# ubisoft/ubisoft-laforge-msmd

Hardware: AMD Instinct MI355X
Metric: FLAME frames/sec on 4s@16kHz clips (whole job; MSMD.forward motion-coefficient frames) (higher is better)
Workload: dtype bf16; 1 GPU; configs[1]: MSMD.forward, batch=32 x 4 s clips per GPU, wav2vec2-base encoder + 8-layer motion decoder, eval-mode, synthetic closed-form weights; batch_per_gpu=32, frames_per_clip=100, parallelism=dp1 (independent clips, no collective), launch=one hipGraph replay per step (the batch sits in the captured input buffers)

## Files before the change

### include/msmd_hip.h

```cpp
#ifndef MSMD_HIP_H
#define MSMD_HIP_H

#include <stdint.h>

#ifdef __cplusplus
extern "C" {
#endif

#define MSMD_F32 0
#define MSMD_BF16 1
#define MSMD_F16 2
#define MSMD_F16X2 3

#define MSMD_ACT_NONE 0
#define MSMD_ACT_GELU 1
#define MSMD_ACT_ELU 2

typedef void* msmd_stream_t;

int msmd_abi_version(void);
#define MSMD_GEMM_VARIANT(v) ((v) << 8)
#define MSMD_GEMM_WRITE_THROUGH (1 << 16)
#define MSMD_GEMM_PAIRED_STORES (1 << 17)
#define MSMD_GEMM_STAGGER (1 << 18)
#define MSMD_GEMM_ONE_TILE_PER_WORKGROUP (1 << 19)
#define MSMD_GEMM_NO_256_TILE (1 << 20)
#define MSMD_GEMM_W_BELOW_32 (1 << 21)

int msmd_spin_us(float us, long* ticks_out, msmd_stream_t stream);

int msmd_gemm(const void* A, const void* W, const float* bias, const void* residual, void* C,
              int M, int N, int K, int in_dtype, int out_dtype,
              long lda, int rows_per_batch, long a_batch_stride, long ldw, long ldc, long ldr, int act,
              int batch, long strideA, long strideW, long strideC, long strideBias, long strideR,
              msmd_stream_t stream);

int msmd_gemm_ln(const void* A, const void* W, const float* bias, const void* residual, void* C, int M, int N, int K,
                 int in_dtype, int out_dtype, long lda, long ldw, long ldc, long ldr, int act, const float* a_stats,
                 const float* w_colsum, const float* r_stats, const float* r_gamma, const float* r_beta,
                 float* stats_out, int slab_in, int slab_out, float eps, msmd_stream_t stream);

int msmd_gemm_ex(const void* A, const void* W, const float* bias, const void* residual, void* C, int M, int N, int K,
                 int in_dtype, int out_dtype, long lda, int rows_per_batch, long a_batch_stride, long ldw, long ldc,
                 long ldr, int act, int batch, long strideA, long strideW, long strideC, long strideBias, long strideR,
                 void* z_out, float p_drop, const unsigned long* rng_state, unsigned int site, msmd_stream_t stream);

int msmd_gemm_route(const void* A, const void* W, const float* bias, const void* residual, void* C, int M, int N, int K,
                    int in_dtype, int out_dtype, long lda, int rows_per_batch, long a_batch_stride, long ldw, long ldc,
                    long ldr, int act, int batch, long strideA, long strideW, long strideC, long strideBias, long strideR,
                    void* z_out, float p_drop, const unsigned long* rng_state, unsigned int site, msmd_stream_t stream);
int msmd_gemm_ln_route(const void* A, const void* W, const float* bias, const void* residual, void* C, int M, int N, int K,
                       int in_dtype, int out_dtype, long lda, long ldw, long ldc, long ldr, int act, const float* a_stats,
                       const float* w_colsum, const float* r_stats, const float* r_gamma, const float* r_beta,
                       float* stats_out, int slab_in, int slab_out, float eps, msmd_stream_t stream);

int msmd_gemm_actbwd(const void* A, const void* W, const void* Z, void* C, int M, int N, int K, int in_dtype, int out_dtype,
                     long lda, long ldw, int act, float p_drop, const unsigned long* rng_state, unsigned int site,
                     msmd_stream_t stream);

int msmd_gemm_batched2(const void* A, const void* W, void* C, int M, int N, int K, int in_dtype, int out_dtype,
                       long lda, long ldw, long ldc, int batch_outer, long strideA_o, long strideW_o, long strideC_o,
                       int batch_inner, long strideA_i, long strideW_i, long strideC_i, msmd_stream_t stream);

int msmd_gemm_tn(const void* A, const void* B, float* C, float* colsum, int M, int N, int K, long lda, long ldb,
                 long ldc, int batch, long strideA, long strideB, long strideC, int b_rows_per_window,
                 long b_window_stride, int accumulate, void* ws, long ws_bytes, msmd_stream_t stream);
long msmd_gemm_tn_workspace(int M, int N, int K, int batch);

int msmd_layernorm(const void* x, const void* residual, const float* gamma, const float* beta,
                   const float* post_add, void* y, int rows, int cols, float eps, int act,
                   int in_dtype, int out_dtype, msmd_stream_t stream);
int msmd_layernorm_pre(const void* x, const float* pre_gamma, const float* pre_beta, const void* residual,
                       const float* gamma, const float* beta, void* y, int rows, int cols, float eps, int dtype,
                       msmd_stream_t stream);

int msmd_layernorm_f16x2(const float* x, const float* residual, const float* gamma, const float* beta,
                         const float* post_add, float* y, void* y_split, int rows, int cols, float eps, int act,
                         msmd_stream_t stream);

int msmd_split_f16x2(const float* x, void* y, long rows, int cols, long ldx, int cols_out, msmd_stream_t stream);
int msmd_unsplit_f16x2(const void* x, float* y, long rows, int cols, int cols_in, long ldy, msmd_stream_t stream);

int msmd_attention_prefetch(const void* Q, const void* K, const void* V, void* O, int B, int H, int Tq, int Tk,
                            long q_bstride, long q_tstride, long k_bstride, long k_tstride, long v_bstride,
                            long v_tstride, long o_bstride, long o_tstride, float scale, const uint8_t* mask, int dtype,
                            const void* const* prefetch_ptrs, const long* prefetch_bytes, int n_prefetch,
                            msmd_stream_t stream);
// ... 273 lines not shown
```

### ubisoft-laforge-msmd_amd/csrc/gemm.hip

```cpp
#include "common.h"
#include <atomic>
#include <utility>

struct GemmArgs {
  const void* A; const void* W; const float* bias; const void* R; void* C;
  int M, N, K;
  long lda; int rows_per_batch; long a_batch_stride; long ldw, ldc, ldr;
  int act; int vec_ok; float inv_rpb;
  long strideA, strideW, strideC, strideBias, strideR;
  int mt, nt;
  int batch_inner; long strideA2, strideW2, strideC2;
  void* Z; float p_drop; const unsigned long* rng; unsigned site;
  int xn;
  int flags;
  const float* a_stats = nullptr; int a_nt = 0; const float* w_colsum = nullptr;
  const float* r_stats = nullptr; int r_nt = 0; const float* r_gamma = nullptr; const float* r_beta = nullptr;
  float* stats_out = nullptr; float ln_eps = 1e-5f;
  int stagger_ticks = 0;
};

enum : int {
  GF_WRITE_THROUGH = 1, GF_PAIRED_STORES = 2, GF_STAGGER = 4,
  GF_ACT_BWD = 8,
  GF_ONE_TILE = 16, GF_NO_256 = 32,
  GF_W_BELOW_32 = 64,
};
struct GemmActWord { int act, hint, flags; };
static constexpr GemmActWord gemm_unpack_act(int act) {
  return {act & 0xff, (act >> 8) & 0xff, ((act >> 16) & 7) | (((act >> 19) & 7) << 4)};
}
static_assert(gemm_unpack_act(MSMD_GEMM_WRITE_THROUGH).flags == GF_WRITE_THROUGH && gemm_unpack_act(MSMD_GEMM_PAIRED_STORES).flags == GF_PAIRED_STORES &&
              gemm_unpack_act(MSMD_GEMM_STAGGER).flags == GF_STAGGER && gemm_unpack_act(MSMD_GEMM_ONE_TILE_PER_WORKGROUP).flags == GF_ONE_TILE &&
              gemm_unpack_act(MSMD_GEMM_NO_256_TILE).flags == GF_NO_256 && gemm_unpack_act(MSMD_GEMM_W_BELOW_32).flags == GF_W_BELOW_32 && gemm_unpack_act(~0).flags == (0x7f & ~GF_ACT_BWD),
              "internal flag bits follow include/msmd_hip.h; no bit of `act` sets the internal one");
enum : int {
  GV_GENERIC = 0,
  GV_SPLIT_128 = 1, GV_SPLIT_64 = 5,
  GV_64_DEEP = 9, GV_64 = 12,
  GV_256x64 = 14,
  GV_192 = 15,
  GV_128 = 17,
  GV_64x128 = 18,
  GV_128_AB = 13, GV_128_ONE_AB = 66,
  GV_256 = 80,
};

enum GemmEpi : int { EPI_ALL = 0, EPI_PLAIN = 1, EPI_LN_OPERAND = 2, EPI_LN_RESIDUAL = 3 };
constexpr int ACT_RUNTIME = -1;
constexpr int epia(GemmEpi e, int act) { return e + 10 * (1 + act); }
constexpr GemmEpi epia_family(int code) { return (GemmEpi)(code % 10); }
constexpr int epia_act(int code) { return code / 10 - 1; }

template <typename T> struct Mfma;
template <> struct Mfma<bf16_t> {
  static __device__ __forceinline__ void run(const u32x4& a, const u32x4& b, f32x4& acc) {
    acc = __builtin_amdgcn_mfma_f32_16x16x32_bf16(__builtin_bit_cast(bf16x8, a), __builtin_bit_cast(bf16x8, b),
                                                  acc, 0, 0, 0);
  }
};
template <> struct Mfma<f16_t> {
  static __device__ __forceinline__ void run(const u32x4& a, const u32x4& b, f32x4& acc) {
    acc = __builtin_amdgcn_mfma_f32_16x16x32_f16(__builtin_bit_cast(f16x8, a), __builtin_bit_cast(f16x8, b), acc, 0, 0, 0);
  }
};
template <> struct Mfma<float> {
  static __device__ __forceinline__ void run(const u32x4& a, const u32x4& b, f32x4& acc) {
#pragma unroll
// ... 208 lines not shown
      }
    }
  }
}

template <int FM>
__device__ __forceinline__ void ln_issue(const float* stats, int nt, int M, int m_base, int fr, int fq, f32x2 (&raw)[FM][4]) {
#pragma unroll
  for (int j = 0; j < FM; ++j) {
    const f32x2* sp = (const f32x2*)stats + min(m_base + j * 16 + fr, M - 1);
#pragma unroll
    for (int q = 0; q < 4; ++q) raw[j][q] = fq + 4 * q < nt ? sp[(long)(fq + 4 * q) * M] : f32x2{0.f, 0.f};
  }
}

template <int FM>
__device__ __forceinline__ void ln_finish(const float* stats, int nt, int M, int m_base, int fr, int fq, const f32x2 (&raw)[FM][4],
                                          float inv_cols, float eps, float (&mu)[FM], float (&rs)[FM]) {
#pragma unroll
  for (int j = 0; j < FM; ++j) {
    float S = (raw[j][0][0] + raw[j][1][0]) + (raw[j][2][0] + raw[j][3][0]);
    float Q = (raw[j][0][1] + raw[j][1][1]) + (raw[j][2][1] + raw[j][3][1]);
    if (nt > 16) {
      const f32x2* sp = (const f32x2*)stats + min(m_base + j * 16 + fr, M - 1);
      for (int t = 16 + fq; t < nt; t += 4) { const f32x2 w = sp[(long)t * M]; S += w[0]; Q += w[1]; }
    }
    S += __shfl_xor(S, 16, 64); S += __shfl_xor(S, 32, 64);
    Q += __shfl_xor(Q, 16, 64); Q += __shfl_xor(Q, 32, 64);
    mu[j] = S * inv_cols;
    rs[j] = rsqrtf(fmaxf(Q * inv_cols - mu[j] * mu[j], 0.f) + eps);
  }
}

template <typename TO, int FM, int FN> struct LnResOps { f32x4 bv[FN], xv[FN], yv[FN]; typename Vec4T<TO>::type rr[FM][FN]; };
template <typename TO, int FM, int FN>
__device__ __forceinline__ void ln_res_issue(const GemmArgs& p, int m_base, int n_base, int fr, int fq, LnResOps<TO, FM, FN>& o) {
  typedef typename Vec4T<TO>::type V4;
  const int n = n_base + fq * 4;
#pragma unroll
  for (int i = 0; i < FN; ++i) o.bv[i] = *(const f32x4*)(p.bias + n + i * 16);
#pragma unroll
  for (int j = 0; j < FM; ++j) {
    const TO* rp = (const TO*)p.R + (long)min(m_base + j * 16 + fr, p.M - 1) * p.ldr + n;
#pragma unroll
    for (int i = 0; i < FN; ++i) o.rr[j][i] = *(const V4*)(rp + i * 16);
  }
  if (p.r_stats) {
#pragma unroll
    for (int i = 0; i < FN; ++i) { o.xv[i] = *(const f32x4*)(p.r_gamma + n + i * 16); o.yv[i] = *(const f32x4*)(p.r_beta + n + i * 16); }
  } else {
#pragma unroll
    for (int i = 0; i < FN; ++i) { o.xv[i] = f32x4{1.f, 1.f, 1.f, 1.f}; o.yv[i] = f32x4{0.f, 0.f, 0.f, 0.f}; }
  }
}

template <typename TO, int FM, int FN, int MODE, int ACT = -1, bool EARLY = false>
__device__ __forceinline__ void gemm_epilogue_ln(const GemmArgs& p, const f32x4 (&acc)[FN][FM], int m_base, int n_base,
                                                 int fr, int fq, const f32x2 (&raw)[FM][4], const LnResOps<TO, FM, FN>* early = nullptr) {
  static_assert((FN == 4 || FN == 2) && (FM >= 2 && FM <= 4), "one wave = one statistics slab of 16 FN columns, 2 to 4 fragment rows");
  constexpr int SLAB = FN * 16;
  constexpr int IB = FM == 3 ? 2 : FN;
  typedef typename Vec4T<TO>::type V4;
  const int n = n_base + fq * 4;
  float mu[FM], rs[FM];
#pragma unroll
  for (int j = 0; j < FM; ++j) { mu[j] = 0.f; rs[j] = 1.f; }
  if constexpr (MODE == 1) ln_finish<FM>(p.a_stats, p.a_nt, p.M, m_base, fr, fq, raw, 1.0f / (float)p.K, p.ln_eps, mu, rs);
  else if (p.r_stats) ln_finish<FM>(p.r_stats, p.r_nt, p.M, m_base, fr, fq, raw, 1.0f / (float)p.N, p.ln_eps, mu, rs);
  float rowS[FM], rowQ[FM], tS[FM], tQ[FM], prS[FM], prQ[FM];
#pragma unroll
  for (int j = 0; j < FM; ++j) rowS[j] = rowQ[j] = tS[j] = tQ[j] = prS[j] = prQ[j] = 0.f;
  const bool odd = fq & 1;
  const bool pair = sizeof(TO) == 2 && (p.flags & GF_PAIRED_STORES);
#pragma unroll
  for (int i0 = 0; i0 < FN; i0 += IB) {
    f32x4 bv[IB], xv[IB], yv[IB];
    V4 rr[FM][IB];
    if constexpr (EARLY) {
      static_assert(MODE == 2 && IB == FN, "the early operands are the LayerNorm-residual form's, all fragment columns at once");
#pragma unroll
      for (int ii = 0; ii < IB; ++ii) {
        bv[ii] = early->bv[ii]; xv[ii] = early->xv[ii]; yv[ii] = early->yv[ii];
#pragma unroll
        for (int j = 0; j < FM; ++j) rr[j][ii] = early->rr[j][ii];
      }
    } else {
#pragma unroll
      for (int ii = 0; ii < IB; ++ii) bv[ii] = *(const f32x4*)(p.bias + n + (i0 + ii) * 16);
      if constexpr (MODE == 1) {
#pragma unroll
        for (int ii = 0; ii < IB; ++ii) xv[ii] = *(const f32x4*)(p.w_colsum + n + (i0 + ii) * 16);
      } else {
#pragma unroll
        for (int j = 0; j < FM; ++j) {
          const TO* rp = (const TO*)p.R + (long)min(m_base + j * 16 + fr, p.M - 1) * p.ldr + n;
#pragma unroll
          for (int ii = 0; ii < IB; ++ii) rr[j][ii] = *(const V4*)(rp + (i0 + ii) * 16);
        }
        if (p.r_stats) {
#pragma unroll
          for (int ii = 0; ii < IB; ++ii) { xv[ii] = *(const f32x4*)(p.r_gamma + n + (i0 + ii) * 16); yv[ii] = *(const f32x4*)(p.r_beta + n + (i0 + ii) * 16); }
        } else {
#pragma unroll
          for (int ii = 0; ii < IB; ++ii) { xv[ii] = f32x4{1.f, 1.f, 1.f, 1.f}; yv[ii] = f32x4{0.f, 0.f, 0.f, 0.f}; }
        }
      }
    }
#pragma unroll
    for (int ii = 0; ii < IB; ++ii) {
      const int i = i0 + ii;
      V4 o[FM];
#pragma unroll
      for (int j = 0; j < FM; ++j) {
        float v[4];
#pragma unroll
        for (int e = 0; e < 4; ++e) {
          float x = acc[i][j][e];
// ... 126 lines not shown
    for (int j = 0; j < FM; ++j) acc[i][j] = f32x4{0.f, 0.f, 0.f, 0.f};

  const int nk = (p.K + BKE - 1) / BKE;
  load_global(0);
  store_lds(0);
  __syncthreads();
  for (int kt = 0; kt < nk; ++kt) {
    const int cur = kt & 1;
    if (kt + 1 < nk) load_global((kt + 1) * BKE);
    const unsigned char* sa = smem + cur * (BM + BN) * 128;
    const unsigned char* sw = sa + BM * 128;
#pragma unroll
    for (int g = 0; g < 2; ++g) {
      u32x4 fx[FM], fw[FN];
#pragma unroll
      for (int j = 0; j < FM; ++j) fx[j] = *(const u32x4*)(sa + lds_off(wm + j * 16 + fr, g * 4 + fq));
#pragma unroll
      for (int i = 0; i < FN; ++i) fw[i] = *(const u32x4*)(sw + lds_off(wn + i * 16 + fr, g * 4 + fq));
#pragma unroll
      for (int i = 0; i < FN; ++i)
#pragma unroll
        for (int j = 0; j < FM; ++j) Mfma<T>::run(fw[i], fx[j], acc[i][j]);
    }
    if (kt + 1 < nk) store_lds(cur ^ 1);
    __syncthreads();
  }

  gemm_epilogue<TO, FM, FN>(p, acc, z, m0 + wm, n0 + wn, fr, fq);
}

typedef __attribute__((address_space(3))) void lds_void_t;
typedef __attribute__((address_space(1))) const void gbl_void_t;

template <typename TO, int BM, int BN, int WM, int WN, int NSTAGE, bool PIPE = false, typename TI = bf16_t, int EPIA = 0>
__global__ __launch_bounds__(WM * WN * 64, (WM * WN == 8 && NSTAGE * (BM + BN) * 128 <= 80 * 1024 && (epia_family(EPIA) != EPI_ALL || BM * BN <= 128 * 128)) ? 4 : 1) void gemm2_kernel(const GemmArgs p) {
  constexpr int EPI = epia_family(EPIA), ACTK = epia_act(EPIA);
  constexpr int NW = WM * WN, NT = NW * 64;
  constexpr int STAGE = (BM + BN) * 128;
  constexpr int LPT = (BM + BN) * 8 / NT;
  constexpr int FM = BM / WM / 16, FN = BN / WN / 16;
  static_assert((BM + BN) * 8 % NT == 0, "tile chunks must divide over the threads");
  extern __shared__ __attribute__((aligned(16))) unsigned char smem[];

  const int pid = blockIdx.x;
  const int xcd = pid & 7, slot = pid >> 3;
  const int xm_n = 8 / p.xn, ntx = (p.nt + p.xn - 1) / p.xn;
  const int m_tile = (slot / ntx) * xm_n + (xcd % xm_n), n_tile = (slot % ntx) * p.xn + xcd / xm_n;
  if (m_tile >= p.mt || n_tile >= p.nt) return;
  const int z = blockIdx.z;
  const int zo = z / p.batch_inner, zi = z % p.batch_inner;
  const bf16_t* __restrict__ A = (const bf16_t*)p.A + zo * p.strideA + zi * p.strideA2;
  const bf16_t* __restrict__ W = (const bf16_t*)p.W + zo * p.strideW + zi * p.strideW2;
  const int m0 = m_tile * BM, n0 = n_tile * BN;
  const int tid = threadIdx.x, lane = tid & 63, wid = tid >> 6;

  const bf16_t* src[LPT];
#pragma unroll
  for (int i = 0; i < LPT; ++i) {
    const int id = (i * NW + wid) * 64 + lane;
    const int row = id >> 3, phys = id & 7;
    const int c = phys ^ ((row >> 1) & 7);
    if (row < BM) {
      const int m = min(m0 + row, p.M - 1);
      src[i] = A + a_row_offset(p, m) + c * 8;
    } else {
      const int n = min(n0 + row - BM, p.N - 1);
      src[i] = W + (long)n * p.ldw + c * 8;
    }
  }
  auto issue = [&](int kt, int stage) {
#pragma unroll
    for (int i = 0; i < LPT; ++i)
      __builtin_amdgcn_global_load_lds((gbl_void_t*)(src[i] + kt * 64),
                                       (lds_void_t*)(smem + stage * STAGE + (i * NW + wid) * 1024), 16, 0, 0);
  };

  const int wm = (wid / WN) * (BM / WM), wn = (wid % WN) * (BN / WN);
  const int fr = lane & 15, fq = lane >> 4;
  f32x4 acc[FN][FM];
#pragma unroll
  for (int i = 0; i < FN; ++i)
#pragma unroll
    for (int j = 0; j < FM; ++j) acc[i][j] = f32x4{0.f, 0.f, 0.f, 0.f};

  const int nk = p.K / 64;
  constexpr bool LNK = (BN == 128 || BN == 64) && WN == 2 && (FM == 2 || FM == 3) && sizeof(TO) == 2;
  constexpr bool LN_LATE = FM == 3;
  constexpr bool EARLY_OPS = LNK && EPI == 3 && NW == 4 && BM == 64 && BN == 128;
  f32x2 lnraw[(LNK && !LN_LATE) ? FM : 1][4];
  std::conditional_t<EARLY_OPS, LnResOps<TO, FM, FN>, char> early;
  (void)early;
  if constexpr (EARLY_OPS) {
    if (p.r_stats) ln_issue<FM>(p.r_stats, p.r_nt, p.M, m0 + wm, fr, fq, lnraw);
    ln_res_issue<TO, FM, FN>(p, m0 + wm, n0 + wn, fr, fq, early);
  }
#pragma unroll
  for (int s = 0; s < NSTAGE - 1; ++s)
    if (s < nk) issue(s, s);
  if (p.stagger_ticks > 0 && ((pid >> 8) & 1) && pid < 512) {
    const unsigned long t0 = __builtin_amdgcn_s_memrealtime();
    while ((long)(__builtin_amdgcn_s_memrealtime() - t0) < p.stagger_ticks) __builtin_amdgcn_s_sleep(16);
  }
  if constexpr (LNK && !LN_LATE && EPI != 1 && !EARLY_OPS) {
    if (EPI == 2 || (EPI == 0 && p.a_stats)) ln_issue<FM>(p.a_stats, p.a_nt, p.M, m0 + wm, fr, fq, lnraw);
    else if (p.r_stats) ln_issue<FM>(p.r_stats, p.r_nt, p.M, m0 + wm, fr, fq, lnraw);
  }
  int stage = 0;
  for (int kt = 0; kt < nk; ++kt) {
    if (kt + NSTAGE - 2 < nk) asm volatile("s_waitcnt vmcnt(%0)" ::"n"((NSTAGE - 2) * LPT) : "memory");
    else asm volatile("s_waitcnt vmcnt(0)" ::: "memory");
    __builtin_amdgcn_s_barrier();
    if (kt + NSTAGE - 1 < nk) issue(kt + NSTAGE - 1, (stage + NSTAGE - 1) % NSTAGE);
    const unsigned char* sa = smem + stage * STAGE;
    const unsigned char* sw = sa + BM * 128;
    if constexpr (PIPE) {
      u32x4 fx[2][FM], fw[2][FN];
#pragma unroll
      for (int g = 0; g < 2; ++g) {
#pragma unroll
        for (int j = 0; j < FM; ++j) fx[g][j] = *(const u32x4*)(sa + lds_off(wm + j * 16 + fr, g * 4 + fq));
#pragma unroll
        for (int i = 0; i < FN; ++i) fw[g][i] = *(const u32x4*)(sw + lds_off(wn + i * 16 + fr, g * 4 + fq));
      }
      __builtin_amdgcn_sched_barrier(0);
#pragma unroll
      for (int g = 0; g < 2; ++g) {
#pragma unroll
        for (int i = 0; i < FN; ++i)
#pragma unroll
          for (int j = 0; j < FM; ++j) Mfma<TI>::run(fw[g][i], fx[g][j], acc[i][j]);
        __builtin_amdgcn_sched_barrier(0);
      }
    } else {
#pragma unroll
      for (int g = 0; g < 2; ++g) {
        u32x4 fx[FM], fw[FN];
#pragma unroll
        for (int j = 0; j < FM; ++j) fx[j] = *(const u32x4*)(sa + lds_off(wm + j * 16 + fr, g * 4 + fq));
#pragma unroll
        for (int i = 0; i < FN; ++i) fw[i] = *(const u32x4*)(sw + lds_off(wn + i * 16 + fr, g * 4 + fq));
#pragma unroll
        for (int i = 0; i < FN; ++i)
#pragma unroll
          for (int j = 0; j < FM; ++j) Mfma<TI>::run(fw[i], fx[j], acc[i][j]);
      }
    }
    stage = (stage + 1 == NSTAGE) ? 0 : stage + 1;
  }
  int tid_e = tid;
  if constexpr (LN_LATE) asm volatile("" : "+v"(tid_e));
  const int wm_e = ((tid_e >> 6) / WN) * (BM / WM), wn_e = ((tid_e >> 6) % WN) * (BN / WN);
  const int fr_e = tid_e & 15, fq_e = (tid_e & 63) >> 4;
  auto run_epilogue = [&]() {
    if constexpr (EPI == 1) { gemm_epilogue<TO, FM, FN, false, true, ACTK>(p, acc, z, m0 + wm_e, n0 + wn_e, fr_e, fq_e); return; }
    if constexpr (LNK && !LN_LATE && EPI == 2) { gemm_epilogue_ln<TO, FM, FN, 1, ACTK>(p, acc, m0 + wm_e, n0 + wn_e, fr_e, fq_e, lnraw); return; }
    if constexpr (EARLY_OPS) { gemm_epilogue_ln<TO, FM, FN, 2, ACTK, true>(p, acc, m0 + wm_e, n0 + wn_e, fr_e, fq_e, lnraw, &early); return; }
    if constexpr (LNK && !LN_LATE && EPI == 3) { gemm_epilogue_ln<TO, FM, FN, 2, ACTK>(p, acc, m0 + wm_e, n0 + wn_e, fr_e, fq_e, lnraw); return; }
    if constexpr (LNK && LN_LATE && (EPI == 2 || EPI == 3)) {
      f32x2 late[FM][4];
      if constexpr (EPI == 2) ln_issue<FM>(p.a_stats, p.a_nt, p.M, m0 + wm_e, fr_e, fq_e, late);
      else if (p.r_stats) ln_issue<FM>(p.r_stats, p.r_nt, p.M, m0 + wm_e, fr_e, fq_e, late);
      gemm_epilogue_ln<TO, FM, FN, EPI - 1, ACTK>(p, acc, m0 + wm_e, n0 + wn_e, fr_e, fq_e, late);
      return;
    }
    if constexpr (LNK && !LN_LATE) {
      if (p.a_stats) { gemm_epilogue_ln<TO, FM, FN, 1, ACTK>(p, acc, m0 + wm_e, n0 + wn_e, fr_e, fq_e, lnraw); return; }
      if (p.r_stats || p.stats_out) { gemm_epilogue_ln<TO, FM, FN, 2, ACTK>(p, acc, m0 + wm_e, n0 + wn_e, fr_e, fq_e, lnraw); return; }
    }
    if constexpr (LNK && LN_LATE) {
      if (p.a_stats || p.r_stats || p.stats_out) {
        f32x2 late[FM][4];
        if (p.a_stats) ln_issue<FM>(p.a_stats, p.a_nt, p.M, m0 + wm_e, fr_e, fq_e, late);
        else if (p.r_stats) ln_issue<FM>(p.r_stats, p.r_nt, p.M, m0 + wm_e, fr_e, fq_e, late);
        if (p.a_stats) gemm_epilogue_ln<TO, FM, FN, 1, ACTK>(p, acc, m0 + wm_e, n0 + wn_e, fr_e, fq_e, late);
        else gemm_epilogue_ln<TO, FM, FN, 2, ACTK>(p, acc, m0 + wm_e, n0 + wn_e, fr_e, fq_e, late);
        return;
      }
    }
    gemm_epilogue<TO, FM, FN, sizeof(TO) == 2, false, ACTK>(p, acc, z, m0 + wm_e, n0 + wn_e, fr_e, fq_e);
  };
  run_epilogue();
}

template <typename TO, int BM, int BN, int WM, int WN, typename TI, int EPIA>
__global__ __launch_bounds__(WM * WN * 64, 4) void gemm2p_kernel(const GemmArgs p) {
  constexpr int EPI = epia_family(EPIA), ACTK = epia_act(EPIA);
  constexpr int NW = WM * WN, NT = NW * 64;
  constexpr int STAGE = (BM + BN) * 128;
  constexpr int LPT = (BM + BN) * 8 / NT;
// ... 716 lines not shown
  return r;
}

template <auto KFN>
static int gemm_launch_kernel(dim3 grid, int threads, int lds, hipStream_t st, const GemmArgs& p) {
  if (lds > 0) {
    static std::atomic<unsigned long> allowed{0};
    int dev = 0;
    (void)hipGetDevice(&dev);
    const unsigned long bit = (unsigned)dev < 64 ? 1UL << dev : 0;
    if (!(allowed.load(std::memory_order_relaxed) & bit)) {
      (void)hipFuncSetAttribute((const void*)KFN, hipFuncAttributeMaxDynamicSharedMemorySize, lds);
      allowed.fetch_or(bit, std::memory_order_relaxed);
    }
  }
  hipLaunchKernelGGL(KFN, grid, dim3(threads), lds, st, p);
  MSMD_RETURN_LAST();
}

static int gemm2_xcd_grid(GemmArgs& p, int BM, int BN, long lda) {
  p.mt = (p.M + BM - 1) / BM; p.nt = (p.N + BN - 1) / BN;
  const double a_bytes = 2.0 * p.M * (double)(p.rows_per_batch < p.M ? lda : p.K), w_bytes = 2.0 * p.N * (double)p.K;
  double best = 1e30;
  int want_xn = 1;
  for (int xn = 1; xn <= 4; xn *= 2) {
    const double c = 0.7 * xn * a_bytes + (8.0 / xn) * w_bytes;
    if (c < best && p.nt >= xn) { best = c; want_xn = xn; }
  }
  p.xn = p.nt >= want_xn ? want_xn : 1;
  const int xm_n = 8 / p.xn;
  return ((p.mt + xm_n - 1) / xm_n) * ((p.nt + p.xn - 1) / p.xn) * 8;
}

template <typename TO, int BM, int BN, int WM, int WN, int NSTAGE, bool PIPE = false, typename TI = bf16_t, int EPIA = 0>
static int launch_gemm2(GemmArgs& p, int wgs, int batch, hipStream_t st) {
  constexpr int lds = NSTAGE * (BM + BN) * 128;
  p.stagger_ticks = ((p.flags & GF_STAGGER) && batch == 1 && lds <= 80 * 1024 && (long)p.mt * p.nt > 640)
                        ? (int)(100.0 * 0.5 * ((p.K / 64) * 0.5 + 3.0)) : 0;
  return gemm_launch_kernel<gemm2_kernel<TO, BM, BN, WM, WN, NSTAGE, PIPE, TI, EPIA>>(dim3(wgs, 1, batch), WM * WN * 64, lds, st, p);
}

static int gemm_epia(const GemmArgs& p, bool lnk) {
  GemmEpi e = EPI_ALL;
  if (lnk && p.a_stats) e = EPI_LN_OPERAND;
  else if (lnk && (p.r_stats || p.stats_out)) e = EPI_LN_RESIDUAL;
  else if (!p.a_stats && !p.r_stats && !p.stats_out && !p.Z && !(p.p_drop > 0.f) && !(p.flags & GF_ACT_BWD)) e = EPI_PLAIN;
  return epia(e, p.act == MSMD_ACT_NONE ? MSMD_ACT_NONE : (p.act == MSMD_ACT_GELU && e != EPI_LN_RESIDUAL) ? MSMD_ACT_GELU : ACT_RUNTIME);
}

template <typename TO, int BM, int BN, int WM, int WN, int NSTAGE, bool PIPE = false, typename TI = bf16_t>
static int launch_gemm2_epi(GemmArgs& p, int batch, hipStream_t st) {
  constexpr bool LNK = (BN == 128 || BN == 64) && WN == 2 && (BM / WM / 16 == 2 || BM / WM / 16 == 3) && sizeof(TO) == 2;
  const int code = gemm_epia(p, LNK), wgs = gemm2_xcd_grid(p, BM, BN, p.lda);
  int r;
  if constexpr (LNK && PIPE && NSTAGE == 2 && WM * WN == 8 && BN == 128 && BM == 128) {
    if (batch == 1 && wgs > 512 && !(p.flags & GF_ONE_TILE)) {
      auto persistent = [&](auto c) { return gemm_launch_kernel<gemm2p_kernel<TO, BM, BN, WM, WN, TI, decltype(c)::value>>(dim3(512), WM * WN * 64, 2 * (BM + BN) * 128, st, p); };
      if ((r = dispatch_code<11, 21, 12, 22>(code, persistent)) >= 0) return r;
    }
  }
  auto run = [&](auto c) { return launch_gemm2<TO, BM, BN, WM, WN, NSTAGE, PIPE, TI, decltype(c)::value>(p, wgs, batch, st); };
  if constexpr (LNK) {
    if ((r = dispatch_code<2, 12, 22, 3, 13>(code, run)) >= 0) return r;
  }
  if ((r = dispatch_code<1, 11, 21>(code, run)) >= 0) return r;
  if constexpr (__is_same(TI, bf16_t)) {
    if ((r = dispatch_code<10, 20>(code, run)) >= 0) return r;
  }
  return run(std::integral_constant<int, 0>{});
}

static int gemm8_workgroup_cap() {
  int dev = 0, n = 0;
  if (hipGetDevice(&dev) != hipSuccess || hipDeviceGetAttribute(&n, hipDeviceAttributeMultiprocessorCount, dev) != hipSuccess || n <= 0) n = 256;
  return n;
}

static long gemm_last_row_offset(const GemmArgs& p) {
  return p.rows_per_batch < p.M ? ((long)((p.M - 1) / p.rows_per_batch) * p.a_batch_stride + (long)(p.rows_per_batch - 1) * p.lda) : (long)(p.M - 1) * p.lda;
}

static bool gemm8_takes(const GemmArgs& p, int batch, int osz) {
  if (osz != 2 || batch != 1 || p.batch_inner != 1 || (p.N % 256) || (p.K % 64) || p.K < 128 || !p.vec_ok) return false;
  if (p.Z || p.p_drop > 0.f || (p.flags & GF_ACT_BWD)) return false;
  if (((uintptr_t)p.bias & 15) || ((uintptr_t)p.C & 7) || ((uintptr_t)p.R & 7)) return false;
  if ((gemm_last_row_offset(p) + p.K) * 2 >= (1L << 32) || ((long)(p.N - 1) * p.ldw + p.K) * 2 >= (1L << 32)) return false;
  const GemmEpi epi = epia_family(gemm_epia(p, true));
  if ((p.a_stats || p.r_stats) && ((p.M & 1) || ((uintptr_t)p.a_stats & 15) || ((uintptr_t)p.r_stats & 15))) return false;
// ... 233 lines not shown
                             const unsigned long* rng_state, unsigned int site) {
  GemmCall c;
  c.A = A; c.W = W; c.bias = bias; c.residual = residual; c.C = C;
  c.M = M; c.N = N; c.K = K; c.in_dtype = in_dtype; c.out_dtype = out_dtype;
  c.lda = lda; c.rows_per_batch = rows_per_batch; c.a_batch_stride = a_batch_stride; c.ldw = ldw; c.ldc = ldc; c.ldr = ldr;
  c.act = act; c.batch = batch;
  c.strideA = strideA; c.strideW = strideW; c.strideC = strideC; c.strideBias = strideBias; c.strideR = strideR;
  c.z_out = z_out; c.p_drop = p_drop; c.rng = rng_state; c.site = site;
  return c;
}

extern "C" int msmd_gemm_ex(const void* A, const void* W, const float* bias, const void* residual, void* C, int M, int N, int K, int in_dtype,
                            int out_dtype, long lda, int rows_per_batch, long a_batch_stride, long ldw, long ldc, long ldr, int act, int batch,
                            long strideA, long strideW, long strideC, long strideBias, long strideR, void* z_out, float p_drop,
                            const unsigned long* rng_state, unsigned int site, msmd_stream_t stream) {
  return gemm_run(gemm_plan, gemm_ex_call(A, W, bias, residual, C, M, N, K, in_dtype, out_dtype, lda, rows_per_batch, a_batch_stride, ldw, ldc, ldr,
                                          act, batch, strideA, strideW, strideC, strideBias, strideR, z_out, p_drop, rng_state, site), stream);
}

extern "C" int msmd_gemm(const void* A, const void* W, const float* bias, const void* residual, void* C, int M, int N, int K, int in_dtype,
                         int out_dtype, long lda, int rows_per_batch, long a_batch_stride, long ldw, long ldc, long ldr, int act, int batch,
                         long strideA, long strideW, long strideC, long strideBias, long strideR, msmd_stream_t stream) {
  return msmd_gemm_ex(A, W, bias, residual, C, M, N, K, in_dtype, out_dtype, lda, rows_per_batch, a_batch_stride, ldw, ldc, ldr,
                      act, batch, strideA, strideW, strideC, strideBias, strideR, nullptr, 0.f, nullptr, 0, stream);
}

extern "C" int msmd_gemm_route(const void* A, const void* W, const float* bias, const void* residual, void* C, int M, int N, int K, int in_dtype,
                               int out_dtype, long lda, int rows_per_batch, long a_batch_stride, long ldw, long ldc, long ldr, int act, int batch,
                               long strideA, long strideW, long strideC, long strideBias, long strideR, void* z_out, float p_drop,
                               const unsigned long* rng_state, unsigned int site, msmd_stream_t) {
  GemmArgs p;
  return gemm_plan(p, gemm_ex_call(A, W, bias, residual, C, M, N, K, in_dtype, out_dtype, lda, rows_per_batch, a_batch_stride, ldw, ldc, ldr,
                                   act, batch, strideA, strideW, strideC, strideBias, strideR, z_out, p_drop, rng_state, site));
}

static int gemm_ln_plan(GemmArgs& p, const GemmCall& c) {
  const int M = c.M, N = c.N, K = c.K;
  if (M <= 0 || N <= 0 || K <= 0 || !c.A || !c.W || !c.C || (K % 64) || (N % 64)) return -1;
  if ((c.in_dtype != MSMD_BF16 && c.in_dtype != MSMD_F16) || c.out_dtype != c.in_dtype) return -1;
  if ((c.lda % 8) || (c.ldw % 8) || (c.ldc % 4) || (c.residual && (c.ldr % 4))) return -1;
  if (((uintptr_t)c.A & 15) || ((uintptr_t)c.W & 15) || ((uintptr_t)c.C & 15) || ((uintptr_t)c.residual & 7) || ((uintptr_t)c.bias & 15)) return -1;
  if ((c.a_stats != nullptr) != (c.w_colsum != nullptr)) return -1;
  if (!c.bias || (c.a_stats && (c.residual || c.stats_out)) || (!c.a_stats && !c.residual)) return -1;
  if (c.r_stats && (!c.residual || !c.r_gamma || !c.r_beta || c.a_stats)) return -1;
  if (((uintptr_t)c.w_colsum & 15) || ((uintptr_t)c.r_gamma & 15) || ((uintptr_t)c.r_beta & 15)) return -1;
  if (((uintptr_t)c.a_stats & 7) || ((uintptr_t)c.r_stats & 7) || ((uintptr_t)c.stats_out & 7)) return -1;
  if ((c.a_stats || c.r_stats) && c.slab_in != 32 && c.slab_in != 64) return -1;
  if (c.stats_out && c.slab_out != 32 && c.slab_out != 64) return -1;
  if ((c.a_stats && (K % c.slab_in)) || (c.r_stats && (N % c.slab_in))) return -1;
  const long tiles128 = (long)((M + 127) / 128) * ((N + 127) / 128);
  const int cols = (c.stats_out ? c.slab_out == 64 : (tiles128 >= 192 && (N % 128) == 0)) ? 128 : 64;
  if (cols == 128 && (N % 128)) return -1;
  const GemmActWord u = gemm_unpack_act(c.act);
  p = gemm_args(c, u.act, GF_PAIRED_STORES | (u.flags & GF_ONE_TILE), 2);
  p.a_stats = c.a_stats; p.a_nt = c.a_stats ? K / c.slab_in : 0; p.w_colsum = c.w_colsum;
  p.r_stats = c.r_stats; p.r_nt = c.r_stats ? N / c.slab_in : 0; p.r_gamma = c.r_gamma; p.r_beta = c.r_beta;
  p.stats_out = c.stats_out; p.ln_eps = c.eps;
  const int variant = gemm16_route(p, 1, 2, c.in_dtype == MSMD_BF16, u.hint, u.flags & GF_NO_256, cols);
  return variant != GV_GENERIC ? variant : -1;
}

static GemmCall gemm_ln_call(const void* A, const void* W, const float* bias, const void* residual, void* C, int M, int N, int K, int in_dtype,
                             int out_dtype, long lda, long ldw, long ldc, long ldr, int act, const float* a_stats, const float* w_colsum,
                             const float* r_stats, const float* r_gamma, const float* r_beta, float* stats_out, int slab_in, int slab_out, float eps) {
  GemmCall c;
  c.A = A; c.W = W; c.bias = bias; c.residual = residual; c.C = C;
  c.M = M; c.N = N; c.K = K; c.in_dtype = in_dtype; c.out_dtype = out_dtype;
  c.lda = lda; c.ldw = ldw; c.ldc = ldc; c.ldr = ldr; c.act = act;
  c.a_stats = a_stats; c.w_colsum = w_colsum; c.r_stats = r_stats; c.r_gamma = r_gamma; c.r_beta = r_beta;
  c.stats_out = stats_out; c.slab_in = slab_in; c.slab_out = slab_out; c.eps = eps;
  return c;
}

extern "C" int msmd_gemm_ln(const void* A, const void* W, const float* bias, const void* residual, void* C, int M, int N, int K, int in_dtype,
                            int out_dtype, long lda, long ldw, long ldc, long ldr, int act, const float* a_stats, const float* w_colsum,
                            const float* r_stats, const float* r_gamma, const float* r_beta, float* stats_out, int slab_in, int slab_out,
                            float eps, msmd_stream_t stream) {
  return gemm_run(gemm_ln_plan, gemm_ln_call(A, W, bias, residual, C, M, N, K, in_dtype, out_dtype, lda, ldw, ldc, ldr, act, a_stats,
                                             w_colsum, r_stats, r_gamma, r_beta, stats_out, slab_in, slab_out, eps), stream);
}

extern "C" int msmd_gemm_ln_route(const void* A, const void* W, const float* bias, const void* residual, void* C, int M, int N, int K,
                                  int in_dtype, int out_dtype, long lda, long ldw, long ldc, long ldr, int act, const float* a_stats,
                                  const float* w_colsum, const float* r_stats, const float* r_gamma, const float* r_beta, float* stats_out,
                                  int slab_in, int slab_out, float eps, msmd_stream_t) {
  GemmArgs p;
  return gemm_ln_plan(p, gemm_ln_call(A, W, bias, residual, C, M, N, K, in_dtype, out_dtype, lda, ldw, ldc, ldr, act, a_stats,
                                      w_colsum, r_stats, r_gamma, r_beta, stats_out, slab_in, slab_out, eps));
}

extern "C" int msmd_gemm_actbwd(const void* A, const void* W, const void* Z, void* C, int M, int N, int K, int in_dtype, int out_dtype, long lda,
                                long ldw, int act, float p_drop, const unsigned long* rng_state, unsigned int site, msmd_stream_t stream) {
  if (!Z || in_dtype != out_dtype || (in_dtype != MSMD_BF16 && in_dtype != MSMD_F16) || (N & 3) || ((uintptr_t)Z & 7)) return 1;
  if (K % 64) return 1;
  GemmCall c;
  c.A = A; c.W = W; c.C = C; c.M = M; c.N = N; c.K = K; c.in_dtype = in_dtype; c.out_dtype = out_dtype;
  c.lda = lda; c.ldw = ldw; c.ldc = N; c.act = act & (0xffff | MSMD_GEMM_WRITE_THROUGH | MSMD_GEMM_PAIRED_STORES);
  c.z_out = const_cast<void*>(Z); c.p_drop = p_drop; c.rng = rng_state; c.site = site; c.internal_flags = GF_ACT_BWD;
  return gemm_run(gemm_plan, c, stream);
}

extern "C" int msmd_gemm_batched2(const void* A, const void* W, void* C, int M, int N, int K, int in_dtype, int out_dtype, long lda, long ldw,
                                  long ldc, int batch_outer, long strideA_o, long strideW_o, long strideC_o, int batch_inner, long strideA_i,
                                  long strideW_i, long strideC_i, msmd_stream_t stream) {
  GemmCall c;
  c.A = A; c.W = W; c.C = C; c.M = M; c.N = N; c.K = K; c.in_dtype = in_dtype; c.out_dtype = out_dtype;
  c.lda = lda; c.ldw = ldw; c.ldc = ldc; c.act = MSMD_ACT_NONE;
  c.batch = batch_outer; c.strideA = strideA_o; c.strideW = strideW_o; c.strideC = strideC_o;
  c.batch_inner = batch_inner; c.strideA2 = strideA_i; c.strideW2 = strideW_i; c.strideC2 = strideC_i;
  return gemm_run(gemm_plan, c, stream);
}
```

### ubisoft-laforge-msmd_amd/ops.py

```python
from __future__ import annotations

import ctypes
import os

import torch
from torch.autograd.function import once_differentiable

from . import _lib

F32, BF16, F16, F16X2 = 0, 1, 2, 3
SPLIT = "f16x2"


class Split:
    __slots__ = ("t", "below_32")
    dtype = SPLIT
    is_cuda = True

    def __init__(self, t, below_32=False):
        if t.dtype != torch.float16 or t.shape[-1] % 64 or t.stride(-1) != 1:
            raise TypeError("Split wraps an fp16 tensor whose last dim is 2 x (a multiple of 32)")
        self.t = t
        self.below_32 = below_32

# ... 99 lines not shown
    if t.dtype == torch.float32:
        return F32
    if t.dtype == torch.bfloat16:
        return BF16
    if t.dtype == torch.float16:
        return F16
    raise TypeError(f"unsupported dtype {t.dtype}")


def _p(t):
    return None if t is None else t.data_ptr()


def _stream():
    return torch.cuda.current_stream().cuda_stream


def _need_cuda(*ts):
    for t in ts:
        if isinstance(t, Split):
            t = t.t
        if t is not None and not t.is_cuda:
            raise RuntimeError("msmd_amd ops need tensors on the MI355X (cuda) device; there is no CPU path")


GEMM_AUTOTUNE = os.environ.get("MSMD_GEMM_AUTOTUNE", "0") == "1"
_TUNE_MIN_FLOP = 1.0e9
_TUNE_CANDIDATES = (17, 13, 9, 12)
_TUNED = {}
GEMM_WRITE_THROUGH, GEMM_PAIRED_STORES, GEMM_STAGGER = 1 << 16, 1 << 17, 1 << 18
GEMM_ONE_TILE_PER_WORKGROUP = 1 << 19
GEMM_NO_256_TILE = 1 << 20
GEMM_W_BELOW_32 = 1 << 21
GEMM_LN_FLAGS = 0
GEMM_LN_ROUTER = None
GEMM_LN_ALL_IN_ONE = False


class capture_guard:

    def __enter__(self):
        import gc
        gc.collect()
        self.was = gc.isenabled()
        gc.disable()
        return self

    def __exit__(self, *exc):
        import gc
        if self.was:
            gc.enable()
        return False
PREFETCH_WEIGHTS = os.environ.get("MSMD_PREFETCH", "1") != "0"
FOLD_LN = os.environ.get("MSMD_FOLD_LN", "1") != "0"
GEMM_ROUTER = None
_GEMM_DEFAULT = {"variant": 0, "flags": GEMM_PAIRED_STORES, "split_variant": 0}
if os.environ.get("MSMD_GEMM_ONE_TILE", "0") == "1":
    _GEMM_DEFAULT["flags"] |= GEMM_ONE_TILE_PER_WORKGROUP
    GEMM_LN_FLAGS = GEMM_ONE_TILE_PER_WORKGROUP


if os.environ.get("MSMD_GEMM_NO_256", "0") == "1":
    _GEMM_DEFAULT["flags"] |= GEMM_NO_256_TILE
    GEMM_LN_FLAGS |= GEMM_NO_256_TILE


# ... 1336 lines not shown
```

Measured before the change: 876,100 frames/s.

## Add 160-row tile for LayerNorm-residual GEMM to fit grid in one round

Adds a 160x128 tile variant (10 waves, 4 stages) for the LayerNorm-residual GEMM path. It is picked automatically when a 128-row tiling would need more than 256 workgroups and the 160-row grid fits in one round. The loader is generalised so only a subset of waves issue global-to-LDS loads when the chunk count does not divide evenly. Gamma/beta loads are deferred to the epilogue for this variant to save registers. The aim is to avoid a partial second wave of workgroups, at the cost of a larger tile and fewer loader threads, and a query entry point for the row tile is added.

```diff
diff --git a/include/msmd_hip.h b/include/msmd_hip.h
--- a/include/msmd_hip.h
+++ b/include/msmd_hip.h
@@ -26,6 +26,8 @@
 #define MSMD_GEMM_ONE_TILE_PER_WORKGROUP (1 << 19)
 #define MSMD_GEMM_NO_256_TILE (1 << 20)
 #define MSMD_GEMM_W_BELOW_32 (1 << 21)
+#define MSMD_GEMM_NO_160_ROW_TILE (1 << 22)
+#define MSMD_GEMM_FORCE_160_ROW_TILE (1 << 23)
 
 int msmd_spin_us(float us, long* ticks_out, msmd_stream_t stream);
 
@@ -53,6 +55,10 @@
                        int in_dtype, int out_dtype, long lda, long ldw, long ldc, long ldr, int act, const float* a_stats,
                        const float* w_colsum, const float* r_stats, const float* r_gamma, const float* r_beta,
                        float* stats_out, int slab_in, int slab_out, float eps, msmd_stream_t stream);
+int msmd_gemm_ln_rows(const void* A, const void* W, const float* bias, const void* residual, void* C, int M, int N, int K,
+                      int in_dtype, int out_dtype, long lda, long ldw, long ldc, long ldr, int act, const float* a_stats,
+                      const float* w_colsum, const float* r_stats, const float* r_gamma, const float* r_beta,
+                      float* stats_out, int slab_in, int slab_out, float eps, msmd_stream_t stream);
 
 int msmd_gemm_actbwd(const void* A, const void* W, const void* Z, void* C, int M, int N, int K, int in_dtype, int out_dtype,
                      long lda, long ldw, int act, float p_drop, const unsigned long* rng_state, unsigned int site,
diff --git a/ubisoft-laforge-msmd_amd/csrc/gemm.hip b/ubisoft-laforge-msmd_amd/csrc/gemm.hip
--- a/ubisoft-laforge-msmd_amd/csrc/gemm.hip
+++ b/ubisoft-laforge-msmd_amd/csrc/gemm.hip
@@ -24,15 +24,19 @@
   GF_ACT_BWD = 8,
   GF_ONE_TILE = 16, GF_NO_256 = 32,
   GF_W_BELOW_32 = 64,
+  GF_NO_160 = 128, GF_FORCE_160 = 256,
+  GF_ROWS_160 = 512,
 };
 struct GemmActWord { int act, hint, flags; };
 static constexpr GemmActWord gemm_unpack_act(int act) {
-  return {act & 0xff, (act >> 8) & 0xff, ((act >> 16) & 7) | (((act >> 19) & 7) << 4)};
+  return {act & 0xff, (act >> 8) & 0xff, ((act >> 16) & 7) | (((act >> 19) & 31) << 4)};
 }
 static_assert(gemm_unpack_act(MSMD_GEMM_WRITE_THROUGH).flags == GF_WRITE_THROUGH && gemm_unpack_act(MSMD_GEMM_PAIRED_STORES).flags == GF_PAIRED_STORES &&
               gemm_unpack_act(MSMD_GEMM_STAGGER).flags == GF_STAGGER && gemm_unpack_act(MSMD_GEMM_ONE_TILE_PER_WORKGROUP).flags == GF_ONE_TILE &&
-              gemm_unpack_act(MSMD_GEMM_NO_256_TILE).flags == GF_NO_256 && gemm_unpack_act(MSMD_GEMM_W_BELOW_32).flags == GF_W_BELOW_32 && gemm_unpack_act(~0).flags == (0x7f & ~GF_ACT_BWD),
-              "internal flag bits follow include/msmd_hip.h; no bit of `act` sets the internal one");
+              gemm_unpack_act(MSMD_GEMM_NO_256_TILE).flags == GF_NO_256 && gemm_unpack_act(MSMD_GEMM_W_BELOW_32).flags == GF_W_BELOW_32 &&
+              gemm_unpack_act(MSMD_GEMM_NO_160_ROW_TILE).flags == GF_NO_160 && gemm_unpack_act(MSMD_GEMM_FORCE_160_ROW_TILE).flags == GF_FORCE_160 &&
+              gemm_unpack_act(~0).flags == (0x1ff & ~GF_ACT_BWD),
+              "internal flag bits follow include/msmd_hip.h; no bit of `act` sets the internal ones");
 enum : int {
   GV_GENERIC = 0,
   GV_SPLIT_128 = 1, GV_SPLIT_64 = 5,
@@ -307,9 +311,9 @@
   }
 }
 
-template <typename TO, int FM, int FN> struct LnResOps { f32x4 bv[FN], xv[FN], yv[FN]; typename Vec4T<TO>::type rr[FM][FN]; };
-template <typename TO, int FM, int FN>
-__device__ __forceinline__ void ln_res_issue(const GemmArgs& p, int m_base, int n_base, int fr, int fq, LnResOps<TO, FM, FN>& o) {
+template <typename TO, int FM, int FN, bool GB = true> struct LnResOps { f32x4 bv[FN], xv[GB ? FN : 1], yv[GB ? FN : 1]; typename Vec4T<TO>::type rr[FM][FN]; };
+template <typename TO, int FM, int FN, bool GB>
+__device__ __forceinline__ void ln_res_issue(const GemmArgs& p, int m_base, int n_base, int fr, int fq, LnResOps<TO, FM, FN, GB>& o) {
   typedef typename Vec4T<TO>::type V4;
   const int n = n_base + fq * 4;
 #pragma unroll
@@ -320,18 +324,20 @@
 #pragma unroll
     for (int i = 0; i < FN; ++i) o.rr[j][i] = *(const V4*)(rp + i * 16);
   }
-  if (p.r_stats) {
-#pragma unroll
-    for (int i = 0; i < FN; ++i) { o.xv[i] = *(const f32x4*)(p.r_gamma + n + i * 16); o.yv[i] = *(const f32x4*)(p.r_beta + n + i * 16); }
-  } else {
-#pragma unroll
-    for (int i = 0; i < FN; ++i) { o.xv[i] = f32x4{1.f, 1.f, 1.f, 1.f}; o.yv[i] = f32x4{0.f, 0.f, 0.f, 0.f}; }
-  }
-}
-
-template <typename TO, int FM, int FN, int MODE, int ACT = -1, bool EARLY = false>
+  if constexpr (GB) {
+    if (p.r_stats) {
+#pragma unroll
+      for (int i = 0; i < FN; ++i) { o.xv[i] = *(const f32x4*)(p.r_gamma + n + i * 16); o.yv[i] = *(const f32x4*)(p.r_beta + n + i * 16); }
+    } else {
+#pragma unroll
+      for (int i = 0; i < FN; ++i) { o.xv[i] = f32x4{1.f, 1.f, 1.f, 1.f}; o.yv[i] = f32x4{0.f, 0.f, 0.f, 0.f}; }
+    }
+  }
+}
+
+template <typename TO, int FM, int FN, int MODE, int ACT = -1, bool EARLY = false, bool EARLY_GB = true>
 __device__ __forceinline__ void gemm_epilogue_ln(const GemmArgs& p, const f32x4 (&acc)[FN][FM], int m_base, int n_base,
-                                                 int fr, int fq, const f32x2 (&raw)[FM][4], const LnResOps<TO, FM, FN>* early = nullptr) {
+                                                 int fr, int fq, const f32x2 (&raw)[FM][4], const LnResOps<TO, FM, FN, EARLY_GB>* early = nullptr) {
   static_assert((FN == 4 || FN == 2) && (FM >= 2 && FM <= 4), "one wave = one statistics slab of 16 FN columns, 2 to 4 fragment rows");
   constexpr int SLAB = FN * 16;
   constexpr int IB = FM == 3 ? 2 : FN;
@@ -355,9 +361,19 @@
       static_assert(MODE == 2 && IB == FN, "the early operands are the LayerNorm-residual form's, all fragment columns at once");
 #pragma unroll
       for (int ii = 0; ii < IB; ++ii) {
-        bv[ii] = early->bv[ii]; xv[ii] = early->xv[ii]; yv[ii] = early->yv[ii];
+        bv[ii] = early->bv[ii];
+        if constexpr (EARLY_GB) { xv[ii] = early->xv[ii]; yv[ii] = early->yv[ii]; }
 #pragma unroll
         for (int j = 0; j < FM; ++j) rr[j][ii] = early->rr[j][ii];
+      }
+      if constexpr (!EARLY_GB) {
+        if (p.r_stats) {
+#pragma unroll
+          for (int ii = 0; ii < IB; ++ii) { xv[ii] = *(const f32x4*)(p.r_gamma + n + ii * 16); yv[ii] = *(const f32x4*)(p.r_beta + n + ii * 16); }
+        } else {
+#pragma unroll
+          for (int ii = 0; ii < IB; ++ii) { xv[ii] = f32x4{1.f, 1.f, 1.f, 1.f}; yv[ii] = f32x4{0.f, 0.f, 0.f, 0.f}; }
+        }
       }
     } else {
 #pragma unroll
@@ -550,14 +566,21 @@
 typedef __attribute__((address_space(3))) void lds_void_t;
 typedef __attribute__((address_space(1))) const void gbl_void_t;
 
+constexpr int gemm2_loader_waves(int slots, int waves) {
+  int w = waves;
+  while (slots % w) --w;
+  return w;
+}
+
 template <typename TO, int BM, int BN, int WM, int WN, int NSTAGE, bool PIPE = false, typename TI = bf16_t, int EPIA = 0>
 __global__ __launch_bounds__(WM * WN * 64, (WM * WN == 8 && NSTAGE * (BM + BN) * 128 <= 80 * 1024 && (epia_family(EPIA) != EPI_ALL || BM * BN <= 128 * 128)) ? 4 : 1) void gemm2_kernel(const GemmArgs p) {
   constexpr int EPI = epia_family(EPIA), ACTK = epia_act(EPIA);
-  constexpr int NW = WM * WN, NT = NW * 64;
+  constexpr int NW = WM * WN;
   constexpr int STAGE = (BM + BN) * 128;
-  constexpr int LPT = (BM + BN) * 8 / NT;
+  constexpr int NLW = gemm2_loader_waves((BM + BN) / 8, NW);
+  constexpr int LPT = (BM + BN) / 8 / NLW;
   constexpr int FM = BM / WM / 16, FN = BN / WN / 16;
-  static_assert((BM + BN) * 8 % NT == 0, "tile chunks must divide over the threads");
+  static_assert((BM + BN) % 8 == 0 && NLW * LPT * 8 == BM + BN && (NLW == NW || NLW * 2 > NW), "tile chunks must divide over the loader waves");
   extern __shared__ __attribute__((aligned(16))) unsigned char smem[];
 
   const int pid = blockIdx.x;
@@ -575,7 +598,7 @@
   const bf16_t* src[LPT];
 #pragma unroll
   for (int i = 0; i < LPT; ++i) {
-    const int id = (i * NW + wid) * 64 + lane;
+    const int id = (i * NLW + wid) * 64 + lane;
     const int row = id >> 3, phys = id & 7;
     const int c = phys ^ ((row >> 1) & 7);
     if (row < BM) {
@@ -586,11 +609,13 @@
       src[i] = W + (long)n * p.ldw + c * 8;
     }
   }
+  const bool loader = NLW == NW || __builtin_amdgcn_readfirstlane(wid) < NLW;
   auto issue = [&](int kt, int stage) {
+    if constexpr (NLW != NW) { if (!loader) return; }
 #pragma unroll
     for (int i = 0; i < LPT; ++i)
       __builtin_amdgcn_global_load_lds((gbl_void_t*)(src[i] + kt * 64),
-                                       (lds_void_t*)(smem + stage * STAGE + (i * NW + wid) * 1024), 16, 0, 0);
+                                       (lds_void_t*)(smem + stage * STAGE + (i * NLW + wid) * 1024), 16, 0, 0);
   };
 
   const int wm = (wid / WN) * (BM / WM), wn = (wid % WN) * (BN / WN);
@@ -604,13 +629,14 @@
   const int nk = p.K / 64;
   constexpr bool LNK = (BN == 128 || BN == 64) && WN == 2 && (FM == 2 || FM == 3) && sizeof(TO) == 2;
   constexpr bool LN_LATE = FM == 3;
-  constexpr bool EARLY_OPS = LNK && EPI == 3 && NW == 4 && BM == 64 && BN == 128;
+  constexpr bool EARLY_OPS = LNK && EPI == 3 && ((NW == 4 && BM == 64) || (NW == 10 && BM == 160)) && BN == 128;
   f32x2 lnraw[(LNK && !LN_LATE) ? FM : 1][4];
-  std::conditional_t<EARLY_OPS, LnResOps<TO, FM, FN>, char> early;
+  constexpr bool EARLY_GB = NW == 4;
+  std::conditional_t<EARLY_OPS, LnResOps<TO, FM, FN, EARLY_GB>, char> early;
   (void)early;
   if constexpr (EARLY_OPS) {
     if (p.r_stats) ln_issue<FM>(p.r_stats, p.r_nt, p.M, m0 + wm, fr, fq, lnraw);
-    ln_res_issue<TO, FM, FN>(p, m0 + wm, n0 + wn, fr, fq, early);
+    ln_res_issue<TO, FM, FN, EARLY_GB>(p, m0 + wm, n0 + wn, fr, fq, early);
   }
 #pragma unroll
   for (int s = 0; s < NSTAGE - 1; ++s)
@@ -672,7 +698,7 @@
   auto run_epilogue = [&]() {
     if constexpr (EPI == 1) { gemm_epilogue<TO, FM, FN, false, true, ACTK>(p, acc, z, m0 + wm_e, n0 + wn_e, fr_e, fq_e); return; }
     if constexpr (LNK && !LN_LATE && EPI == 2) { gemm_epilogue_ln<TO, FM, FN, 1, ACTK>(p, acc, m0 + wm_e, n0 + wn_e, fr_e, fq_e, lnraw); return; }
-    if constexpr (EARLY_OPS) { gemm_epilogue_ln<TO, FM, FN, 2, ACTK, true>(p, acc, m0 + wm_e, n0 + wn_e, fr_e, fq_e, lnraw, &early); return; }
+    if constexpr (EARLY_OPS) { gemm_epilogue_ln<TO, FM, FN, 2, ACTK, true, EARLY_GB>(p, acc, m0 + wm_e, n0 + wn_e, fr_e, fq_e, lnraw, &early); return; }
     if constexpr (LNK && !LN_LATE && EPI == 3) { gemm_epilogue_ln<TO, FM, FN, 2, ACTK>(p, acc, m0 + wm_e, n0 + wn_e, fr_e, fq_e, lnraw); return; }
     if constexpr (LNK && LN_LATE && (EPI == 2 || EPI == 3)) {
       f32x2 late[FM][4];
@@ -1455,6 +1481,17 @@
   return ((p.mt + xm_n - 1) / xm_n) * ((p.nt + p.xn - 1) / p.xn) * 8;
 }
 
+static int gemm160_one_round_grid(GemmArgs& p) {
+  const int wgs = gemm2_xcd_grid(p, 160, 128, p.lda);
+  if (wgs <= 256) return wgs;
+  for (int xn = 1; xn <= 4 && xn <= p.nt; xn *= 2) {
+    const int xm_n = 8 / xn;
+    const int w = ((p.mt + xm_n - 1) / xm_n) * ((p.nt + xn - 1) / xn) * 8;
+    if (w <= 256) { p.xn = xn; return w; }
+  }
+  return 0;
+}
+
 template <typename TO, int BM, int BN, int WM, int WN, int NSTAGE, bool PIPE = false, typename TI = bf16_t, int EPIA = 0>
 static int launch_gemm2(GemmArgs& p, int wgs, int batch, hipStream_t st) {
   constexpr int lds = NSTAGE * (BM + BN) * 128;
@@ -1477,6 +1514,11 @@
   const int code = gemm_epia(p, LNK), wgs = gemm2_xcd_grid(p, BM, BN, p.lda);
   int r;
   if constexpr (LNK && PIPE && NSTAGE == 2 && WM * WN == 8 && BN == 128 && BM == 128) {
+    if (p.flags & GF_ROWS_160) {
+      int wgs160 = gemm160_one_round_grid(p);
+      if (!wgs160) wgs160 = gemm2_xcd_grid(p, 160, 128, p.lda);
+      return launch_gemm2<TO, 160, 128, 5, 2, 4, true, TI, epia(EPI_LN_RESIDUAL, MSMD_ACT_NONE)>(p, wgs160, batch, st);
+    }
     if (batch == 1 && wgs > 512 && !(p.flags & GF_ONE_TILE)) {
       auto persistent = [&](auto c) { return gemm_launch_kernel<gemm2p_kernel<TO, BM, BN, WM, WN, TI, decltype(c)::value>>(dim3(512), WM * WN * 64, 2 * (BM + BN) * 128, st, p); };
       if ((r = dispatch_code<11, 21, 12, 22>(code, persistent)) >= 0) return r;
@@ -1776,6 +1818,15 @@
   GemmArgs p;
   return gemm_plan(p, gemm_ex_call(A, W, bias, residual, C, M, N, K, in_dtype, out_dtype, lda, rows_per_batch, a_batch_stride, ldw, ldc, ldr,
                                    act, batch, strideA, strideW, strideC, strideBias, strideR, z_out, p_drop, rng_state, site));
+}
+
+static bool gemm_ln_takes_160_rows(const GemmArgs& p, int cols, const GemmActWord& u) {
+  if (cols != 128 || p.a_stats || !p.R || p.act != MSMD_ACT_NONE || (u.flags & GF_NO_160)) return false;
+  if (u.flags & GF_FORCE_160) return true;
+  if (u.hint) return false;
+  if ((long)((p.M + 127) / 128) * ((p.N + 127) / 128) <= 256) return false;
+  GemmArgs q = p;
+  return gemm160_one_round_grid(q) > 0;
 }
 
 static int gemm_ln_plan(GemmArgs& p, const GemmCall& c) {
@@ -1801,7 +1852,19 @@
   p.r_stats = c.r_stats; p.r_nt = c.r_stats ? N / c.slab_in : 0; p.r_gamma = c.r_gamma; p.r_beta = c.r_beta;
   p.stats_out = c.stats_out; p.ln_eps = c.eps;
   const int variant = gemm16_route(p, 1, 2, c.in_dtype == MSMD_BF16, u.hint, u.flags & GF_NO_256, cols);
+  if (variant == GV_128 && gemm_ln_takes_160_rows(p, cols, u)) p.flags |= GF_ROWS_160;
   return variant != GV_GENERIC ? variant : -1;
+}
+
+static int gemm_ln_plan_rows(const GemmArgs& p, int variant) {
+  switch (variant) {
+    case GV_64_DEEP: case GV_64: case GV_64x128: return 64;
+    case GV_128: return (p.flags & GF_ROWS_160) ? 160 : 128;
+    case GV_128_AB: case GV_128_ONE_AB: return 128;
+    case GV_192: return 192;
+    case GV_256: case GV_256x64: return 256;
+  }
+  return -1;
 }
 
 static GemmCall gemm_ln_call(const void* A, const void* W, const float* bias, const void* residual, void* C, int M, int N, int K, int in_dtype,
@@ -1833,6 +1896,16 @@
                                       w_colsum, r_stats, r_gamma, r_beta, stats_out, slab_in, slab_out, eps));
 }
 
+extern "C" int msmd_gemm_ln_rows(const void* A, const void* W, const float* bias, const void* residual, void* C, int M, int N, int K,
+                                 int in_dtype, int out_dtype, long lda, long ldw, long ldc, long ldr, int act, const float* a_stats,
+                                 const float* w_colsum, const float* r_stats, const float* r_gamma, const float* r_beta, float* stats_out,
+                                 int slab_in, int slab_out, float eps, msmd_stream_t) {
+  GemmArgs p;
+  const int variant = gemm_ln_plan(p, gemm_ln_call(A, W, bias, residual, C, M, N, K, in_dtype, out_dtype, lda, ldw, ldc, ldr, act, a_stats,
+                                                   w_colsum, r_stats, r_gamma, r_beta, stats_out, slab_in, slab_out, eps));
+  return variant < 0 ? -1 : gemm_ln_plan_rows(p, variant);
+}
+
 extern "C" int msmd_gemm_actbwd(const void* A, const void* W, const void* Z, void* C, int M, int N, int K, int in_dtype, int out_dtype, long lda,
                                 long ldw, int act, float p_drop, const unsigned long* rng_state, unsigned int site, msmd_stream_t stream) {
   if (!Z || in_dtype != out_dtype || (in_dtype != MSMD_BF16 && in_dtype != MSMD_F16) || (N & 3) || ((uintptr_t)Z & 7)) return 1;
diff --git a/ubisoft-laforge-msmd_amd/ops.py b/ubisoft-laforge-msmd_amd/ops.py
--- a/ubisoft-laforge-msmd_amd/ops.py
+++ b/ubisoft-laforge-msmd_amd/ops.py
@@ -155,6 +155,8 @@
 GEMM_ONE_TILE_PER_WORKGROUP = 1 << 19
 GEMM_NO_256_TILE = 1 << 20
 GEMM_W_BELOW_32 = 1 << 21
+GEMM_NO_160_ROW_TILE = 1 << 22
+GEMM_FORCE_160_ROW_TILE = 1 << 23
 GEMM_LN_FLAGS = 0
 GEMM_LN_ROUTER = None
 GEMM_LN_ALL_IN_ONE = False
```

After: 901,400 frames/s, median of 6. +2.9%, better.
